# kris927b/TextBlaster

Measured on AMD Instinct MI355X. Metric: documents/sec through full C4+Gopher+langID pipeline at 1/2/4/8 MI355X, higher is better.
Workload: dtype bf16

## Files before the change

### csrc/common/langid.h

```cpp
#pragma once
#include <cmath>

#include "ucd.h"

namespace tb {

constexpr int kLidLangs = 5;
constexpr int kLidRow = 8;
constexpr int kLidBucketsLog2 = 16;
constexpr uint32_t kLidBuckets = 1u << kLidBucketsLog2;
constexpr int kLidMaxCps = 4096;
constexpr int kLidMaxGrams = 4;
constexpr uint32_t kLidBoundary = 0x20;
constexpr int kLidDim = 32;
constexpr int kLidRowDim = 16;
constexpr int kLidHeadCols = 16;
constexpr int kLidQMax = 255;

TB_HD uint32_t lid_hash(uint32_t a, uint32_t b, uint32_t c, uint32_t d, int n) {
  uint32_t h = 2166136261u ^ (uint32_t)n * 0x9E3779B1u;
  h = (h ^ a) * 16777619u;
  if (n >= 2) h = (h ^ b) * 16777619u;
  if (n >= 3) h = (h ^ c) * 16777619u;
  if (n >= 4) h = (h ^ d) * 16777619u;
  h ^= h >> 15;
  h *= 0x2c1b3c6dU;
  h ^= h >> 12;
  return h & (kLidBuckets - 1);
}

template <class F>
TB_HD int lid_grams_n(uint32_t lm3, uint32_t lm2, uint32_t lm1, uint32_t l0, F&& emit) {
  const uint32_t B = kLidBoundary;
  if (l0) {
    emit(lid_hash(l0, 0, 0, 0, 1), 1);
    emit(lid_hash(lm1 ? lm1 : B, l0, 0, 0, 2), 2);
    if (!lm1) return 2;
    emit(lid_hash(lm2 ? lm2 : B, lm1, l0, 0, 3), 3);
    if (!lm2) return 3;
    emit(lid_hash(lm3 ? lm3 : B, lm2, lm1, l0, 4), 4);
    return 4;
  }
  if (!lm1) return 0;
  emit(lid_hash(lm1, B, 0, 0, 2), 2);
  emit(lid_hash(lm2 ? lm2 : B, lm1, B, 0, 3), 3);
  if (!lm2) return 2;
  emit(lid_hash(lm3 ? lm3 : B, lm2, lm1, B, 4), 4);
  return 3;
}

template <class F>
TB_HD int lid_grams_at(uint32_t lm3, uint32_t lm2, uint32_t lm1, uint32_t l0, F&& emit) {
  return lid_grams_n(lm3, lm2, lm1, l0, [&](uint32_t g, int) { emit(g); });
}

TB_HD double lid_exp(double x) {
  if (!(x > -745.0)) return 0.0;
  const double k = floor(fma(x, 1.4426950408889634, 0.5));
  double r = fma(-k, 6.93147180369123816490e-01, x);
  r = fma(-k, 1.90821492927058770002e-10, r);
  double p = 1.0 / 6227020800.0;
  const double inv[13] = {1.0 / 479001600.0, 1.0 / 39916800.0, 1.0 / 3628800.0, 1.0 / 362880.0, 1.0 / 40320.0,
                          1.0 / 5040.0, 1.0 / 720.0, 1.0 / 120.0, 1.0 / 24.0, 1.0 / 6.0, 0.5, 1.0, 1.0};
#pragma unroll
  for (int i = 0; i < 13; ++i) p = fma(p, r, inv[i]);
  return ldexp(p, (int)k);
}

TB_HD void lid_softmax_decide(const double* logit, int64_t* r) {
  int best = 0;
  for (int l = 1; l < kLidLangs; ++l) if (logit[l] > logit[best]) best = l;
  double den = 0;
  for (int l = 0; l < kLidLangs; ++l) den += lid_exp(logit[l] - logit[best]);
  const double conf = 1.0 / den;
  r[0] = best;
  union { double d; int64_t i; } u;
  u.d = conf;
  r[1] = u.i;
}

TB_HD int lid_block_exp(int64_t smax, int64_t cnt) {
  int e = 0;
  while (e < 30 && (smax << (e + 1)) <= (int64_t)kLidQMax * cnt) ++e;
  return e;
}

TB_HD int32_t lid_quant(int64_t s, int e, int64_t cnt) {
  const bool neg = s < 0;
  const int64_t num = (neg ? -s : s) << e;
  int64_t q = num / cnt;
  const int64_t rem = num - q * cnt;
  if (2 * rem > cnt || (2 * rem == cnt && (q & 1))) ++q;
  return (int32_t)(neg ? -q : q);
}

TB_HD void lid_decide_v3(const double* C, int e, int64_t cnt, double w_scale, const float* bias, int64_t* r) {
  if (cnt <= 0) {
    r[0] = -1;
    r[1] = 0;
    return;
  }
  const double sc = ldexp(w_scale, -e);
  double logit[kLidLangs];
  for (int l = 0; l < kLidLangs; ++l) logit[l] = fma(C[l], sc, (double)bias[l]);
  lid_softmax_decide(logit, r);
}

TB_HD uint16_t lid_bf16_bits(float v) {
  union { float f; uint32_t u; } x;
  x.f = v;
  return (uint16_t)(x.u >> 16);
}

TB_HD uint32_t lid_letter(const UcdView& ucd, const uint8_t* b, uint32_t n, int64_t s) {
  if (s < 0) return 0;
  const uint32_t c0 = b[s];
  if (c0 < 0x80u) {
    const uint32_t l = c0 | 0x20u;
    return (l >= 'a' && l <= 'z') ? l : 0u;
  }
  int len;
  const uint32_t c = utf8_decode(b, (uint32_t)s, n, &len);
  if (!(ucd.props(c) & P_ALPHA)) return 0;
  const uint32_t l = ucd.lower(c);
  return l ? l : c;
}

TB_HD int64_t prev_lead(const uint8_t* b, int64_t s) {
  int64_t k = s - 1;
  while (k >= 0 && !utf8_is_lead(b[k])) --k;
  return k;
}

struct LidTables {
  const float* bias = nullptr;
  const int8_t* E = nullptr;
  const int16_t* W = nullptr;
  double w_scale = 0;
};

TB_HD int lid_half(int n) { return n >= 3 ? kLidRowDim : 0; }

TB_HD void lid_add_emb(const int8_t* E, uint32_t g, int n, int32_t* acc) {
  const int8_t* r = E + (size_t)g * kLidRowDim;
  int32_t* a = acc + lid_half(n);
#pragma unroll
  for (int d = 0; d < kLidRowDim; ++d) a[d] += r[d];
}

TB_HD void lid_record_v3(const int64_t* S, int64_t cnt, const LidTables& lt, int64_t* r) {
  if (cnt <= 0) {
    r[0] = -1;
    r[1] = 0;
    return;
  }
  int64_t smax = 0;
  for (int d = 0; d < kLidDim; ++d) smax = (S[d] < 0 ? -S[d] : S[d]) > smax ? (S[d] < 0 ? -S[d] : S[d]) : smax;
  const int e = lid_block_exp(smax, cnt);
  int32_t a[kLidDim];
  for (int d = 0; d < kLidDim; ++d) a[d] = lid_quant(S[d], e, cnt);
  double C[kLidLangs];
  for (int l = 0; l < kLidLangs; ++l) {
    int64_t c = 0;
    for (int d = 0; d < kLidDim; ++d) c += (int64_t)a[d] * lt.W[d * kLidLangs + l];
    C[l] = (double)c;
  }
  lid_decide_v3(C, e, cnt, lt.w_scale, lt.bias, r);
}

}
```

### csrc/hip/langid.hip

```cpp
#include "kernel_common.h"

namespace {

__device__ __forceinline__ int lid_top(uint64_t m) { return 63 - __clzll((long long)m); }

constexpr int kLidTile = 16;
constexpr int kLidWaves = 8;
typedef __bf16 bf16x8 __attribute__((ext_vector_type(8)));
typedef float f32x4 __attribute__((ext_vector_type(4)));

__device__ __forceinline__ void lid_row_swar(const uint8_t* __restrict__ Eb, uint32_t g, uint32_t* p) {
  const uint4 w = *(const uint4*)(Eb + (size_t)g * kLidRowDim);
  const uint32_t v[4] = {w.x, w.y, w.z, w.w};
#pragma unroll
  for (int q = 0; q < 4; ++q) {
    p[2 * q] += v[q] & 0x00FF00FFu;
    p[2 * q + 1] += (v[q] >> 8) & 0x00FF00FFu;
  }
}

constexpr int kLidSyms = 32;
constexpr int kLidPairs = kLidSyms * kLidSyms;
constexpr uint32_t kLidSymMiss = 32;
constexpr int kLidAuxBytes = kLidPairs * 32 + kLidRowDim;

__device__ __forceinline__ uint32_t lid_sym_letter(int i) {
  if (i == 0) return kLidBoundary;
  if (i <= 26) return 'a' + (uint32_t)(i - 1);
  return i == 27 ? 0xE6 : i == 28 ? 0xF8 : i == 29 ? 0xE5 : i == 30 ? 0xE4 : 0xF6;
}

__device__ __forceinline__ uint32_t lid_sym_latin(uint32_t l) {
  return l == 0xE6 ? 27u : l == 0xF8 ? 28u : l == 0xE5 ? 29u : l == 0xE4 ? 30u : l == 0xF6 ? 31u : kLidSymMiss;
}

__global__ __launch_bounds__(256) void k_lid_pairs(const uint8_t* __restrict__ Eb, uint32_t* __restrict__ aux) {
  const int i = (int)(blockIdx.x * blockDim.x + threadIdx.x);
  if (i < kLidPairs) {
    const int x = i / kLidSyms, y = i % kLidSyms;
    uint32_t d[kLidRowDim];
#pragma unroll
    for (int k = 0; k < kLidRowDim; ++k) d[k] = 0;
    auto add = [&](uint32_t g) {
      for (int k = 0; k < kLidRowDim; ++k) d[k] += Eb[(size_t)g * kLidRowDim + k];
    };
    if (y != 0) add(lid_hash(lid_sym_letter(y), 0, 0, 0, 1));
    if (x != 0 || y != 0) add(lid_hash(lid_sym_letter(x), lid_sym_letter(y), 0, 0, 2));
    for (int q = 0; q < 4; ++q) {
      aux[i * 8 + 2 * q] = d[4 * q] | d[4 * q + 2] << 16;
      aux[i * 8 + 2 * q + 1] = d[4 * q + 1] | d[4 * q + 3] << 16;
    }
  }
  if (i < kLidRowDim / 4) aux[kLidPairs * 8 + i] = 0;
}

__device__ __forceinline__ uint32_t lid_letter_dev(uint32_t cur, const uint8_t* b, uint32_t n, uint32_t s,
                                                   const UcdView& ucd) {
  if (cur < 0x80u) return (cur | 0x20u) - 'a' < 26u ? (cur | 0x20u) : 0u;
  if (cur == 0xC3u && s + 1 < n) {
    const uint32_t c = 0xC0u | (b[s + 1] & 0x3Fu);
    return (c == 0xD7u || c == 0xF7u) ? 0u : (c < 0xDFu ? c | 0x20u : c);
  }
  return lid_letter(ucd, b, n, s);
}

__device__ __forceinline__ void lid_add_u8(uint4 w, uint32_t* p) {
  const uint32_t v[4] = {w.x, w.y, w.z, w.w};
#pragma unroll
  for (int q = 0; q < 4; ++q) {
    p[2 * q] += v[q] & 0x00FF00FFu;
    p[2 * q + 1] += (v[q] >> 8) & 0x00FF00FFu;
  }
}

template <int N>
__device__ __forceinline__ void lid_halve(const int32_t* in, int32_t* out, bool upper, int m) {
#pragma unroll
  for (int j = 0; j < N / 2; ++j) {
    const int32_t keep = upper ? in[N / 2 + j] : in[j];
    const int32_t give = upper ? in[j] : in[N / 2 + j];
    out[j] = keep + __shfl_xor(give, m);
  }
}

__device__ __forceinline__ void lid_fold(uint32_t* pa, uint32_t* pb, int lane, int32_t& dsum) {
  const bool up = (lane >> 5) & 1;
  uint32_t kept[8];
#pragma unroll
  for (int j = 0; j < 8; ++j) {
    const uint32_t keep = up ? pb[j] : pa[j];
    const uint32_t give = up ? pa[j] : pb[j];
    kept[j] = keep + (uint32_t)__shfl_xor((int)give, 32);
    pa[j] = pb[j] = 0;
  }
  int32_t u[16], v8[8], v4[4], v2[2], v1;
#pragma unroll
  for (int j = 0; j < 8; ++j) {
    u[2 * j] = (int32_t)(kept[j] & 0xFFFFu);
    u[2 * j + 1] = (int32_t)(kept[j] >> 16);
  }
  lid_halve<16>(u, v8, (lane >> 4) & 1, 16);
  lid_halve<8>(v8, v4, (lane >> 3) & 1, 8);
  lid_halve<4>(v4, v2, (lane >> 2) & 1, 4);
  lid_halve<2>(v2, &v1, (lane >> 1) & 1, 2);
  dsum += v1 + __shfl_xor(v1, 1);
}

__device__ __forceinline__ void lid_doc_vector(const uint8_t* __restrict__ b, uint32_t n, const UcdView& ucd,
                                               const uint8_t* __restrict__ Eb, const uint8_t* __restrict__ zero,
                                               const uint4* pairs, uint32_t* slot, int lane, uint16_t* arow,
                                               int32_t* e_out, int64_t* cnt_out) {
  uint32_t lim = n;
  if (n > (uint32_t)kLidMaxCps) {
    uint32_t seen = 0;
    for (uint32_t base = 0; base < n; base += 64) {
      const uint32_t i = base + (uint32_t)lane;
      const uint64_t m = __ballot(i < n && utf8_is_lead(b[i]));
      const uint32_t c = (uint32_t)__popcll(m);
      if (seen + c > (uint32_t)kLidMaxCps) {
        uint64_t mm = m;
        for (uint32_t k = seen; k < (uint32_t)kLidMaxCps; ++k) mm &= mm - 1;
        lim = base + (uint32_t)__builtin_ctzll(mm);
        break;
      }
      seen += c;
    }
  }
  uint32_t pa[8] = {0u, 0u, 0u, 0u, 0u, 0u, 0u, 0u}, pb[8] = {0u, 0u, 0u, 0u, 0u, 0u, 0u, 0u};
  int32_t dsum = 0;
  uint32_t cnt_lo = 0, cnt_hi = 0, chunks = 0;
  const uint32_t B = kLidBoundary;
  if (lane < 3) slot[lane] = 0;
  uint8_t cur = (uint32_t)lane < lim ? b[lane] : (uint8_t)0;
  for (uint32_t base = 0; base <= lim; base += 64) {
    const uint32_t s = base + (uint32_t)lane;
    const uint8_t nxt = s + 64 < lim ? b[s + 64] : (uint8_t)0;
    const bool lead = s < lim && utf8_is_lead(cur);
    const bool emit = lead || s == lim;
    uint32_t l0 = 0, y = 0;
    if (lead) {
      l0 = lid_letter_dev(cur, b, n, s, ucd);
      y = l0 < 0x80u ? (l0 & 0x1Fu) : lid_sym_latin(l0);
    }
    const uint64_t M = __ballot(lead);
    const uint64_t EM = __ballot(emit);
    const uint32_t r = __builtin_amdgcn_mbcnt_hi((uint32_t)(EM >> 32), __builtin_amdgcn_mbcnt_lo((uint32_t)EM, 0u));
    if (lead) slot[3 + r] = l0 | y << 24;
    __builtin_amdgcn_fence(__ATOMIC_RELEASE, "wavefront");
    __builtin_amdgcn_wave_barrier();
    __builtin_amdgcn_fence(__ATOMIC_ACQUIRE, "wavefront");
    uint32_t e1 = slot[2 + r], e2 = slot[1 + r], e3 = slot[r];
    if (!emit) e1 = e2 = e3 = 0;
    const uint32_t lm1 = e1 & 0xFFFFFFu, lm2 = e2 & 0xFFFFFFu, lm3 = e3 & 0xFFFFFFu;
    const uint32_t x = e1 >> 24;
    const bool miss = ((x | y) & kLidSymMiss) != 0;
    const uint4* pr = pairs + 2 * (miss ? 0u : (x << 5 | y));
    const uint4 t0 = pr[0], t1 = pr[1];
    pa[0] += t0.x; pa[1] += t0.y; pa[2] += t0.z; pa[3] += t0.w;
    pa[4] += t1.x; pa[5] += t1.y; pa[6] += t1.z; pa[7] += t1.w;
    cnt_lo += (l0 != 0u) + ((l0 | lm1) != 0u);
    if (__ballot(miss)) {
      if (miss) {
        if (l0) lid_add_u8(*(const uint4*)(Eb + (size_t)lid_hash(l0, 0, 0, 0, 1) * kLidRowDim), pa);
        if (l0 | lm1)
          lid_add_u8(*(const uint4*)(Eb + (size_t)lid_hash(lm1 ? lm1 : B, l0 ? l0 : B, 0, 0, 2) * kLidRowDim), pa);
      }
    }
    const uint32_t x0 = l0 ? l0 : B;
    const bool v3 = lm1 != 0u, v4 = v3 && lm2 != 0u;
    const uint8_t* g3 = v3 ? Eb + (size_t)lid_hash(lm2 ? lm2 : B, lm1, x0, 0, 3) * kLidRowDim : zero;
    const uint8_t* g4 = v4 ? Eb + (size_t)lid_hash(lm3 ? lm3 : B, lm2, lm1, x0, 4) * kLidRowDim : zero;
    lid_add_u8(*(const uint4*)g3, pb);
    lid_add_u8(*(const uint4*)g4, pb);
    cnt_hi += (uint32_t)v3 + (uint32_t)v4;
    if ((++chunks & 63u) == 0) lid_fold(pa, pb, lane, dsum);
    const uint32_t c = (uint32_t)__popcll(M);
    uint32_t keep = 0;
    if (lane < 3) keep = slot[c + lane];
    __builtin_amdgcn_fence(__ATOMIC_RELEASE, "wavefront");
    __builtin_amdgcn_wave_barrier();
    __builtin_amdgcn_fence(__ATOMIC_ACQUIRE, "wavefront");
    if (lane < 3) slot[lane] = keep;
    cur = nxt;
  }
  lid_fold(pa, pb, lane, dsum);
  for (int o = 1; o < 64; o <<= 1) {
    cnt_lo += (uint32_t)__shfl_xor((int)cnt_lo, o);
    cnt_hi += (uint32_t)__shfl_xor((int)cnt_hi, o);
  }
  const uint32_t cnt = cnt_lo + cnt_hi;
  const bool up = ((lane >> 5) & 1) != 0;
  const int32_t S = dsum - 128 * (int32_t)(up ? cnt_hi : cnt_lo);
  const int dim = ((lane >> 5) & 1) * 16 + (2 * ((lane >> 4) & 1) + ((lane >> 3) & 1)) * 4 + ((lane >> 2) & 1) +
                  2 * ((lane >> 1) & 1);
  int32_t smax = S < 0 ? -S : S;
  for (int o = 1; o < 64; o <<= 1) {
    const int32_t t = __shfl_xor(smax, o);
    smax = t > smax ? t : smax;
  }
  const int e = cnt ? lid_block_exp((int64_t)smax, (int64_t)cnt) : 0;
  if ((lane & 1) == 0) arow[dim] = cnt ? lid_bf16_bits((float)lid_quant((int64_t)S, e, (int64_t)cnt)) : (uint16_t)0;
  if (lane == 0) {
    *e_out = e;
    *cnt_out = (int64_t)cnt;
  }
}

__global__ __launch_bounds__(64 * kLidWaves) __attribute__((amdgpu_waves_per_eu(8, 8))) void k_langid_mfma(
    const uint8_t* __restrict__ bytes, const int64_t* __restrict__ off, const int32_t* __restrict__ perm,
    int32_t ndocs, DevTables tabs, const uint8_t* __restrict__ Eb, const uint8_t* __restrict__ aux,
    const uint16_t* __restrict__ WT, double w_scale, const float* __restrict__ bias, int64_t* rec, int32_t width,
    uint64_t* prof) {
  __shared__ __attribute__((aligned(16))) uint16_t A[kLidTile][kLidDim];
  __shared__ float Cm[kLidTile][kLidHeadCols];
  __shared__ int32_t ex[kLidTile];
  __shared__ int64_t cn[kLidTile];
  __shared__ uint4 pairs[2 * kLidPairs];
  __shared__ uint32_t slots[kLidWaves][68];
  const int w = (int)(threadIdx.x >> 6), lane = (int)(threadIdx.x & 63);
  const UcdView ucd{tabs.s1, tabs.s2, tabs.l1, tabs.l2};
  for (int i = (int)threadIdx.x; i < 2 * kLidPairs; i += 64 * kLidWaves) pairs[i] = ((const uint4*)aux)[i];
  const uint8_t* zero = aux + kLidPairs * 32;
  __syncthreads();
  const int ntiles = (ndocs + kLidTile - 1) / kLidTile;
  for (int tile = (int)blockIdx.x; tile < ntiles; tile += (int)gridDim.x) {
    for (int r = w; r < kLidTile; r += kLidWaves) {
      const int pos = tile * kLidTile + r;
      const int doc = pos < ndocs ? (perm ? perm[pos] : pos) : -1;
      if (doc < 0) {
        if (lane < kLidDim) A[r][lane] = 0;
        if (lane == 0) {
          ex[r] = 0;
          cn[r] = 0;
        }
        continue;
      }
      const uint64_t t0 = prof ? __builtin_amdgcn_s_memtime() : 0;
      lid_doc_vector(bytes + off[doc], (uint32_t)(off[doc + 1] - off[doc]), ucd, Eb, zero, pairs, slots[w], lane,
                     A[r], &ex[r], &cn[r]);
      if (prof && lane == 0) prof[(size_t)doc * kPhaseSlots + PH_LID] += __builtin_amdgcn_s_memtime() - t0;
    }
    __syncthreads();
    if (w == 0) {
      const bf16x8 a = *reinterpret_cast<const bf16x8*>(&A[lane & 15][8 * (lane >> 4)]);
      const bf16x8 bw = *reinterpret_cast<const bf16x8*>(WT + (lane & 15) * kLidDim + 8 * (lane >> 4));
      f32x4 c = {0.f, 0.f, 0.f, 0.f};
      c = __builtin_amdgcn_mfma_f32_16x16x32_bf16(a, bw, c, 0, 0, 0);
#pragma unroll
      for (int r = 0; r < 4; ++r) Cm[(lane >> 4) * 4 + r][lane & 15] = c[r];
      __builtin_amdgcn_fence(__ATOMIC_RELEASE, "workgroup");
      __builtin_amdgcn_wave_barrier();
      __builtin_amdgcn_fence(__ATOMIC_ACQUIRE, "workgroup");
      const int p2 = tile * kLidTile + lane;
      if (lane < kLidTile && p2 < ndocs) {
        const int d2 = perm ? perm[p2] : p2;
        double C[kLidLangs];
#pragma unroll
        for (int l = 0; l < kLidLangs; ++l) C[l] = (double)Cm[lane][l];
        lid_decide_v3(C, ex[lane], cn[lane], w_scale, bias, rec + (int64_t)d2 * width);
      }
    }
    __syncthreads();
  }
}

}

extern "C" {

int tb_langid_aux_bytes() { return kLidAuxBytes; }
int tb_langid_prepare(hipStream_t stream, const uint8_t* E, uint8_t* aux) {
  if (!E || !aux) return (int)hipErrorInvalidValue;
  hipLaunchKernelGGL(k_lid_pairs, dim3((kLidPairs + 255) / 256), dim3(256), 0, stream, E, (uint32_t*)aux);
  return (int)hipGetLastError();
}

int tb_langid_mfma(hipStream_t stream, const TbDocs* d, const TbTables* tb, const uint8_t* E, const uint8_t* aux,
                   const uint16_t* WT, double w_scale, const float* bias, int64_t* rec, int32_t width,
                   uint64_t* prof) {
  const int32_t ndocs = d->n_launch;
  if (ndocs <= 0) return 0;
  if (!E || !aux || !WT || !bias || !rec || width < 2 || !(w_scale > 0)) return (int)hipErrorInvalidValue;
  const int ntiles = (ndocs + kLidTile - 1) / kLidTile;
  const int cus = device_cus();
  const int grid = ntiles < 4 * cus ? ntiles : 4 * cus;
  hipLaunchKernelGGL(k_langid_mfma, dim3(grid), dim3(64 * kLidWaves), 0, stream, d->bytes, d->off, d->perm, ndocs,
                     tb->ucd, E, aux, WT, w_scale, bias, rec, width, prof);
  return (int)hipGetLastError();
}

}
```

Before: 14.13 million.

## Precompute trigram embedding table and rework langid scan with ballot/bpermute and buffer loads

Adds a precomputed 32^3 symbol-trigram table built at prepare time, so most 3-gram hashes become direct table lookups instead of hash plus random embedding gathers. The per-wave LDS slot exchange with barriers is replaced by ds_bpermute/readlane carry of the previous letters. UTF-8 lead detection now uses ballot-mask arithmetic, ASCII and 2-byte letters go through a 256-entry LDS lookup table, and row loads use bounds-checked buffer loads that return zero out of range, which removes the zero-row pointer trick. It also drops the final count shuffle reduction by counting with popcount on masks. The aux buffer grows (32K trigram rows), and the rewritten position logic brings a correctness risk.

```diff
diff --git a/csrc/common/langid.h b/csrc/common/langid.h
--- a/csrc/common/langid.h
+++ b/csrc/common/langid.h
@@ -148,6 +148,40 @@
   for (int d = 0; d < kLidRowDim; ++d) a[d] += r[d];
 }
 
+constexpr int kLidSyms = 32;
+constexpr uint32_t kLidSymMiss = 32;
+
+TB_HD uint32_t lid_sym_letter(int i) {
+  if (i == 0) return kLidBoundary;
+  if (i <= 26) return 'a' + (uint32_t)(i - 1);
+  return i == 27 ? 0xE6 : i == 28 ? 0xF8 : i == 29 ? 0xE5 : i == 30 ? 0xE4 : 0xF6;
+}
+
+TB_HD uint32_t lid_sym_latin(uint32_t l) {
+  return l == 0xE6 ? 27u : l == 0xF8 ? 28u : l == 0xE5 ? 29u : l == 0xE4 ? 30u : l == 0xF6 ? 31u : kLidSymMiss;
+}
+
+TB_HD uint32_t lid_sym(uint32_t l) { return l < 0x80u ? (l & 0x1Fu) : lid_sym_latin(l); }
+
+template <class T>
+TB_HD void lid_pair_entry(const T* E, int x, int y, int32_t* d) {
+  if (y != 0) {
+    const T* r = E + (size_t)lid_hash(lid_sym_letter(y), 0, 0, 0, 1) * kLidRowDim;
+    for (int k = 0; k < kLidRowDim; ++k) d[k] += (int32_t)r[k];
+  }
+  if (x != 0 || y != 0) {
+    const T* r = E + (size_t)lid_hash(lid_sym_letter(x), lid_sym_letter(y), 0, 0, 2) * kLidRowDim;
+    for (int k = 0; k < kLidRowDim; ++k) d[k] += (int32_t)r[k];
+  }
+}
+
+template <class T>
+TB_HD void lid_tri_entry(const T* E, int s2, int s1, int s0, int32_t* d) {
+  if (s1 == 0) return;
+  const T* r = E + (size_t)lid_hash(lid_sym_letter(s2), lid_sym_letter(s1), lid_sym_letter(s0), 0, 3) * kLidRowDim;
+  for (int k = 0; k < kLidRowDim; ++k) d[k] += (int32_t)r[k];
+}
+
 TB_HD void lid_record_v3(const int64_t* S, int64_t cnt, const LidTables& lt, int64_t* r) {
   if (cnt <= 0) {
     r[0] = -1;
diff --git a/csrc/hip/langid.hip b/csrc/hip/langid.hip
--- a/csrc/hip/langid.hip
+++ b/csrc/hip/langid.hip
@@ -1,6 +1,12 @@
 #include "kernel_common.h"
 
 namespace {
+
+__device__ __forceinline__ uint64_t lid_eq(uint32_t a, uint32_t b) { return __builtin_amdgcn_uicmp(a, b, 32); }
+__device__ __forceinline__ uint64_t lid_ne(uint32_t a, uint32_t b) { return __builtin_amdgcn_uicmp(a, b, 33); }
+__device__ __forceinline__ uint64_t lid_lt(uint32_t a, uint32_t b) { return __builtin_amdgcn_uicmp(a, b, 36); }
+__device__ __forceinline__ uint64_t lid_ge(uint32_t a, uint32_t b) { return __builtin_amdgcn_uicmp(a, b, 35); }
+__device__ __forceinline__ bool lid_on(uint64_t m) { return __builtin_amdgcn_inverse_ballot_w64(m); }
 
 __device__ __forceinline__ int lid_top(uint64_t m) { return 63 - __clzll((long long)m); }
 
@@ -9,49 +15,45 @@
 typedef __bf16 bf16x8 __attribute__((ext_vector_type(8)));
 typedef float f32x4 __attribute__((ext_vector_type(4)));
 
-__device__ __forceinline__ void lid_row_swar(const uint8_t* __restrict__ Eb, uint32_t g, uint32_t* p) {
-  const uint4 w = *(const uint4*)(Eb + (size_t)g * kLidRowDim);
-  const uint32_t v[4] = {w.x, w.y, w.z, w.w};
-#pragma unroll
-  for (int q = 0; q < 4; ++q) {
-    p[2 * q] += v[q] & 0x00FF00FFu;
-    p[2 * q + 1] += (v[q] >> 8) & 0x00FF00FFu;
-  }
-}
-
-constexpr int kLidSyms = 32;
+#ifndef TB_LID_TRI_ROW
+#define TB_LID_TRI_ROW 16
+#endif
+constexpr int kLidTriRow = TB_LID_TRI_ROW;
+static_assert(kLidTriRow == 32 || kLidTriRow == 16, "3-gram row: 32 (pre-split) or 16 (bytes)");
 constexpr int kLidPairs = kLidSyms * kLidSyms;
-constexpr uint32_t kLidSymMiss = 32;
-constexpr int kLidAuxBytes = kLidPairs * 32 + kLidRowDim;
-
-__device__ __forceinline__ uint32_t lid_sym_letter(int i) {
-  if (i == 0) return kLidBoundary;
-  if (i <= 26) return 'a' + (uint32_t)(i - 1);
-  return i == 27 ? 0xE6 : i == 28 ? 0xF8 : i == 29 ? 0xE5 : i == 30 ? 0xE4 : 0xF6;
-}
-
-__device__ __forceinline__ uint32_t lid_sym_latin(uint32_t l) {
-  return l == 0xE6 ? 27u : l == 0xF8 ? 28u : l == 0xE5 ? 29u : l == 0xE4 ? 30u : l == 0xF6 ? 31u : kLidSymMiss;
-}
-
-__global__ __launch_bounds__(256) void k_lid_pairs(const uint8_t* __restrict__ Eb, uint32_t* __restrict__ aux) {
+constexpr int kLidTris = kLidSyms * kLidSyms * kLidSyms;
+constexpr int kLidZeroOff = kLidPairs * 32;
+constexpr int kLidTriOff = kLidZeroOff + 32;
+constexpr int kLidAuxBytes = kLidTriOff + kLidTris * kLidTriRow;
+
+__global__ __launch_bounds__(256) void k_lid_tables(const uint8_t* __restrict__ Eb, uint32_t* __restrict__ aux) {
   const int i = (int)(blockIdx.x * blockDim.x + threadIdx.x);
+  if (i >= kLidPairs + kLidTris) return;
+  int32_t d[kLidRowDim];
+#pragma unroll
+  for (int k = 0; k < kLidRowDim; ++k) d[k] = 0;
+  uint32_t* out;
+  bool split = true;
   if (i < kLidPairs) {
-    const int x = i / kLidSyms, y = i % kLidSyms;
-    uint32_t d[kLidRowDim];
-#pragma unroll
-    for (int k = 0; k < kLidRowDim; ++k) d[k] = 0;
-    auto add = [&](uint32_t g) {
-      for (int k = 0; k < kLidRowDim; ++k) d[k] += Eb[(size_t)g * kLidRowDim + k];
-    };
-    if (y != 0) add(lid_hash(lid_sym_letter(y), 0, 0, 0, 1));
-    if (x != 0 || y != 0) add(lid_hash(lid_sym_letter(x), lid_sym_letter(y), 0, 0, 2));
+    lid_pair_entry(Eb, i / kLidSyms, i % kLidSyms, d);
+    out = aux + i * 8;
+  } else {
+    const int t = i - kLidPairs;
+    lid_tri_entry(Eb, t / kLidPairs, (t / kLidSyms) % kLidSyms, t % kLidSyms, d);
+    out = aux + kLidTriOff / 4 + t * (kLidTriRow / 4);
+    split = kLidTriRow == 32;
+  }
+  if (split) {
     for (int q = 0; q < 4; ++q) {
-      aux[i * 8 + 2 * q] = d[4 * q] | d[4 * q + 2] << 16;
-      aux[i * 8 + 2 * q + 1] = d[4 * q + 1] | d[4 * q + 3] << 16;
-    }
-  }
-  if (i < kLidRowDim / 4) aux[kLidPairs * 8 + i] = 0;
+      out[2 * q] = (uint32_t)d[4 * q] | (uint32_t)d[4 * q + 2] << 16;
+      out[2 * q + 1] = (uint32_t)d[4 * q + 1] | (uint32_t)d[4 * q + 3] << 16;
+    }
+  } else {
+    for (int q = 0; q < 4; ++q)
+      out[q] = (uint32_t)d[4 * q] | (uint32_t)d[4 * q + 1] << 8 | (uint32_t)d[4 * q + 2] << 16 |
+               (uint32_t)d[4 * q + 3] << 24;
+  }
+  if (i < (kLidTriOff - kLidZeroOff) / 4) aux[kLidZeroOff / 4 + i] = 0;
 }
 
 __device__ __forceinline__ uint32_t lid_letter_dev(uint32_t cur, const uint8_t* b, uint32_t n, uint32_t s,
@@ -64,13 +66,77 @@
   return lid_letter(ucd, b, n, s);
 }
 
+__device__ __forceinline__ uint32_t lid_table_entry(uint32_t i, uint32_t* buf, const UcdView& ucd) {
+  const uint32_t c0 = i < 0x80u ? i : (0xC2u | ((i >> 6) & 1u));
+  *buf = c0 | (0x80u | (i & 0x3Fu)) << 8;
+  const uint32_t l = lid_letter_dev(c0, (const uint8_t*)buf, i < 0x80u ? 1u : 2u, 0u, ucd);
+  return l ? (l | lid_sym(l) << 24) : 0u;
+}
+
+constexpr uint32_t kLidNoRow = 0x7FFFFFF0u;
+__device__ __forceinline__ __amdgpu_buffer_rsrc_t lid_rsrc(const uint8_t* p, uint32_t bytes) {
+  return __builtin_amdgcn_make_buffer_rsrc((void*)p, 0, (int)bytes, 0x00027000);
+}
+__device__ __forceinline__ uint4 lid_row(__amdgpu_buffer_rsrc_t r, uint32_t off) {
+  typedef uint32_t u32x4 __attribute__((ext_vector_type(4)));
+  const u32x4 v = __builtin_amdgcn_raw_buffer_load_b128(r, (int)off, 0, 0);
+  return uint4{v.x, v.y, v.z, v.w};
+}
+
+__device__ __forceinline__ uint32_t lid_byte(__amdgpu_buffer_rsrc_t r, uint32_t off) {
+  return __builtin_amdgcn_raw_buffer_load_b8(r, (int)off, 0, 0);
+}
+
+__device__ __forceinline__ uint64_t lid_low(int32_t r) {
+  return r >= 64 ? ~(uint64_t)0 : r <= 0 ? (uint64_t)0 : (((uint64_t)1 << r) - 1);
+}
+
+__device__ __forceinline__ uint64_t lid_positions(uint32_t cur, uint64_t K1, int32_t left, uint64_t& pend) {
+  const uint64_t in = lid_low(left);
+  const uint64_t L2 = lid_eq(cur & 0xE0u, 0xC0u) & lid_low(left - 1);
+  const uint64_t L3 = lid_eq(cur & 0xF0u, 0xE0u) & lid_low(left - 2);
+  const uint64_t L4 = ~(K1 | L2 | L3) & lid_low(left - 3);
+  uint64_t P = in & lid_ne(cur & 0xC0u, 0x80u);
+  uint64_t a = P & (L2 | L3 | L4), b = P & (L3 | L4), c = P & L4;
+  if ((in & ~(pend | a << 1 | b << 2 | c << 3)) != P) {
+    uint64_t cov = pend;
+    P = 0;
+    for (int i = 0; i < 64; ++i) {
+      const uint64_t bit = (uint64_t)1 << i;
+      if (in & ~cov & bit) {
+        P |= bit;
+        cov |= ((L2 | L3 | L4) & bit) << 1 | ((L3 | L4) & bit) << 2 | (L4 & bit) << 3;
+      }
+    }
+    a = P & (L2 | L3 | L4), b = P & (L3 | L4), c = P & L4;
+  }
+  pend = a >> 63 | b >> 62 | c >> 61;
+  return P;
+}
+
 __device__ __forceinline__ void lid_add_u8(uint4 w, uint32_t* p) {
   const uint32_t v[4] = {w.x, w.y, w.z, w.w};
+  uint32_t even, odd;
+  asm("s_mov_b32 %0, 0x0c020c00" : "=s"(even));
+  asm("s_mov_b32 %0, 0x0c030c01" : "=s"(odd));
 #pragma unroll
   for (int q = 0; q < 4; ++q) {
-    p[2 * q] += v[q] & 0x00FF00FFu;
-    p[2 * q + 1] += (v[q] >> 8) & 0x00FF00FFu;
-  }
+    p[2 * q] += __builtin_amdgcn_perm(0u, v[q], even);
+    p[2 * q + 1] += __builtin_amdgcn_perm(0u, v[q], odd);
+  }
+}
+
+__device__ __forceinline__ void lid_add_split(uint4 t0, uint4 t1, uint32_t* p) {
+  p[0] += t0.x; p[1] += t0.y; p[2] += t0.z; p[3] += t0.w;
+  p[4] += t1.x; p[5] += t1.y; p[6] += t1.z; p[7] += t1.w;
+}
+
+__device__ __forceinline__ void lid_add_rows(uint4 r3a, uint4 r3b, uint4 r4, uint32_t* pb) {
+  if (kLidTriRow == 32)
+    lid_add_split(r3a, r3b, pb);
+  else
+    lid_add_u8(r3a, pb);
+  lid_add_u8(r4, pb);
 }
 
 template <int N>
@@ -107,15 +173,19 @@
 }
 
 __device__ __forceinline__ void lid_doc_vector(const uint8_t* __restrict__ b, uint32_t n, const UcdView& ucd,
-                                               const uint8_t* __restrict__ Eb, const uint8_t* __restrict__ zero,
-                                               const uint4* pairs, uint32_t* slot, int lane, uint16_t* arow,
-                                               int32_t* e_out, int64_t* cnt_out) {
+                                               const uint8_t* __restrict__ Eb,
+                                               __amdgpu_buffer_rsrc_t EbR, __amdgpu_buffer_rsrc_t triR,
+                                               const uint4* pairs,
+                                               const uint32_t* ltab, int lane, uint16_t* arow, int32_t* e_out,
+                                               int64_t* cnt_out) {
   uint32_t lim = n;
   if (n > (uint32_t)kLidMaxCps) {
     uint32_t seen = 0;
+    uint64_t pend = 0;
     for (uint32_t base = 0; base < n; base += 64) {
       const uint32_t i = base + (uint32_t)lane;
-      const uint64_t m = __ballot(i < n && utf8_is_lead(b[i]));
+      const uint32_t ci = i < n ? b[i] : 0u;
+      const uint64_t m = lid_positions(ci, lid_lt(ci, 0x80u), (int32_t)(n - base), pend);
       const uint32_t c = (uint32_t)__popcll(m);
       if (seen + c > (uint32_t)kLidMaxCps) {
         uint64_t mm = m;
@@ -125,69 +195,94 @@
       }
       seen += c;
     }
+    lim = (uint32_t)__builtin_amdgcn_readfirstlane((int)lim);
   }
   uint32_t pa[8] = {0u, 0u, 0u, 0u, 0u, 0u, 0u, 0u}, pb[8] = {0u, 0u, 0u, 0u, 0u, 0u, 0u, 0u};
   int32_t dsum = 0;
   uint32_t cnt_lo = 0, cnt_hi = 0, chunks = 0;
+  uint32_t c1 = 0, c2 = 0, c3 = 0;
+  uint64_t pend = 0;
   const uint32_t B = kLidBoundary;
-  if (lane < 3) slot[lane] = 0;
-  uint8_t cur = (uint32_t)lane < lim ? b[lane] : (uint8_t)0;
+  const uint64_t below = ((uint64_t)1 << lane) - 1;
+  const __amdgpu_buffer_rsrc_t docR = lid_rsrc(b, n);
+  uint32_t cur = lid_byte(docR, (uint32_t)lane);
+  uint32_t n0 = lid_byte(docR, 64u);
   for (uint32_t base = 0; base <= lim; base += 64) {
-    const uint32_t s = base + (uint32_t)lane;
-    const uint8_t nxt = s + 64 < lim ? b[s + 64] : (uint8_t)0;
-    const bool lead = s < lim && utf8_is_lead(cur);
-    const bool emit = lead || s == lim;
-    uint32_t l0 = 0, y = 0;
-    if (lead) {
-      l0 = lid_letter_dev(cur, b, n, s, ucd);
-      y = l0 < 0x80u ? (l0 & 0x1Fu) : lid_sym_latin(l0);
-    }
-    const uint64_t M = __ballot(lead);
-    const uint64_t EM = __ballot(emit);
-    const uint32_t r = __builtin_amdgcn_mbcnt_hi((uint32_t)(EM >> 32), __builtin_amdgcn_mbcnt_lo((uint32_t)EM, 0u));
-    if (lead) slot[3 + r] = l0 | y << 24;
-    __builtin_amdgcn_fence(__ATOMIC_RELEASE, "wavefront");
-    __builtin_amdgcn_wave_barrier();
-    __builtin_amdgcn_fence(__ATOMIC_ACQUIRE, "wavefront");
-    uint32_t e1 = slot[2 + r], e2 = slot[1 + r], e3 = slot[r];
-    if (!emit) e1 = e2 = e3 = 0;
-    const uint32_t lm1 = e1 & 0xFFFFFFu, lm2 = e2 & 0xFFFFFFu, lm3 = e3 & 0xFFFFFFu;
-    const uint32_t x = e1 >> 24;
-    const bool miss = ((x | y) & kLidSymMiss) != 0;
-    const uint4* pr = pairs + 2 * (miss ? 0u : (x << 5 | y));
-    const uint4 t0 = pr[0], t1 = pr[1];
-    pa[0] += t0.x; pa[1] += t0.y; pa[2] += t0.z; pa[3] += t0.w;
-    pa[4] += t1.x; pa[5] += t1.y; pa[6] += t1.z; pa[7] += t1.w;
-    cnt_lo += (l0 != 0u) + ((l0 | lm1) != 0u);
-    if (__ballot(miss)) {
-      if (miss) {
+    const uint32_t cur1 = lid_byte(docR, base + 64u + (uint32_t)lane);
+    const uint32_t n01 = lid_byte(docR, base + 128u);
+    const int32_t rem = (int32_t)(lim - base);
+    const int32_t left = (int32_t)(n - base);
+    const uint64_t AS = lid_lt(cur, 0x80u);
+    uint64_t P;
+    {
+      const uint64_t A = lid_ge(cur, 0xC0u), E3 = lid_ge(cur, 0xE0u), F4 = lid_ge(cur, 0xF0u);
+      if (left >= 67 && (pend | A << 1 | E3 << 2 | F4 << 3) == ~(AS | A)) {
+        P = AS | A;
+        pend = A >> 63 | E3 >> 62 | F4 >> 61;
+      } else {
+        P = lid_positions(cur, AS, left, pend);
+      }
+    }
+    const uint64_t M = P & lid_low(rem);
+    const uint64_t EM = M | (lid_low(rem + 1) & ~lid_low(rem));
+    uint32_t nb = lane_next(cur);
+    if (lane == 63) nb = n0;
+    const uint64_t TW = lid_eq(cur & 0xFEu, 0xC2u) & lid_low(left - 1);
+    const uint32_t i2 = ((cur << 6 | (nb & 0x3Fu)) & 0x7Fu) | 0x80u;
+    uint32_t ent = ltab[lid_on(M & AS) ? cur : (lid_on(M & TW) ? i2 : 0u)];
+    const uint64_t G = M & ~AS & ~TW;
+    if (G) {
+      if (lid_on(G)) {
+        const uint32_t l = lid_letter(ucd, b, n, base + (uint32_t)lane);
+        ent = l ? (l | lid_sym(l) << 24) : 0u;
+      }
+    }
+    const uint64_t pm = M & below;
+    const bool hasp = pm != 0;
+    const int pl = (63 - __clzll((long long)pm)) << 2;
+    uint32_t e1 = (uint32_t)__builtin_amdgcn_ds_bpermute(pl, (int)ent);
+    e1 = hasp ? e1 : c1;
+    uint32_t e2 = (uint32_t)__builtin_amdgcn_ds_bpermute(pl, (int)e1);
+    e2 = hasp ? e2 : c2;
+    uint32_t e3 = (uint32_t)__builtin_amdgcn_ds_bpermute(pl, (int)e2);
+    e3 = hasp ? e3 : c3;
+    if (M) {
+      const int t = lid_top(M);
+      c3 = (uint32_t)__builtin_amdgcn_readlane((int)e2, t);
+      c2 = (uint32_t)__builtin_amdgcn_readlane((int)e1, t);
+      c1 = (uint32_t)__builtin_amdgcn_readlane((int)ent, t);
+    }
+    e1 = lid_on(EM) ? e1 : 0u;
+    const uint32_t l0 = ent & 0xFFFFFFu, lm1 = e1 & 0xFFFFFFu, lm2 = e2 & 0xFFFFFFu, lm3 = e3 & 0xFFFFFFu;
+    const uint32_t y = ent >> 24, x = e1 >> 24, s2 = e2 >> 24;
+    const uint64_t L0 = lid_ne(l0, 0u), L1 = lid_ne(lm1, 0u), V4 = L1 & lid_ne(lm2, 0u);
+    const uint64_t MS = lid_ne((x | y) & kLidSymMiss, 0u), MS3 = lid_ne((x | y | s2) & kLidSymMiss, 0u);
+    const uint32_t pi = x << 5 | y;
+    const uint4* pr = pairs + 2 * (lid_on(MS) ? 0u : pi);
+    const uint32_t g3 = (s2 << 10 | pi) * (uint32_t)kLidTriRow;
+    const uint32_t x0 = lid_on(L0) ? l0 : B;
+    const uint32_t g4 = lid_hash(lm3 ? lm3 : B, lm2, lm1, x0, 4) * (uint32_t)kLidRowDim;
+    uint4 q3b = {0u, 0u, 0u, 0u};
+    const uint4 q3a = lid_row(triR, lid_on(L1 & ~MS3) ? g3 : kLidNoRow);
+    if (kLidTriRow == 32) q3b = lid_row(triR, lid_on(L1 & ~MS3) ? g3 + 16u : kLidNoRow);
+    const uint4 q4 = lid_row(EbR, lid_on(V4) ? g4 : kLidNoRow);
+    lid_add_split(pr[0], pr[1], pa);
+    lid_add_rows(q3a, q3b, q4, pb);
+    cnt_lo += (uint32_t)__popcll(L0) + (uint32_t)__popcll(L0 | L1);
+    cnt_hi += (uint32_t)__popcll(L1) + (uint32_t)__popcll(V4);
+    if (MS3) {
+      if (lid_on(MS)) {
         if (l0) lid_add_u8(*(const uint4*)(Eb + (size_t)lid_hash(l0, 0, 0, 0, 1) * kLidRowDim), pa);
         if (l0 | lm1)
-          lid_add_u8(*(const uint4*)(Eb + (size_t)lid_hash(lm1 ? lm1 : B, l0 ? l0 : B, 0, 0, 2) * kLidRowDim), pa);
-      }
-    }
-    const uint32_t x0 = l0 ? l0 : B;
-    const bool v3 = lm1 != 0u, v4 = v3 && lm2 != 0u;
-    const uint8_t* g3 = v3 ? Eb + (size_t)lid_hash(lm2 ? lm2 : B, lm1, x0, 0, 3) * kLidRowDim : zero;
-    const uint8_t* g4 = v4 ? Eb + (size_t)lid_hash(lm3 ? lm3 : B, lm2, lm1, x0, 4) * kLidRowDim : zero;
-    lid_add_u8(*(const uint4*)g3, pb);
-    lid_add_u8(*(const uint4*)g4, pb);
-    cnt_hi += (uint32_t)v3 + (uint32_t)v4;
+          lid_add_u8(*(const uint4*)(Eb + (size_t)lid_hash(lm1 ? lm1 : B, x0, 0, 0, 2) * kLidRowDim), pa);
+      }
+      if (lid_on(MS3 & L1)) lid_add_u8(*(const uint4*)(Eb + (size_t)lid_hash(lm2 ? lm2 : B, lm1, x0, 0, 3) * kLidRowDim), pb);
+    }
     if ((++chunks & 63u) == 0) lid_fold(pa, pb, lane, dsum);
-    const uint32_t c = (uint32_t)__popcll(M);
-    uint32_t keep = 0;
-    if (lane < 3) keep = slot[c + lane];
-    __builtin_amdgcn_fence(__ATOMIC_RELEASE, "wavefront");
-    __builtin_amdgcn_wave_barrier();
-    __builtin_amdgcn_fence(__ATOMIC_ACQUIRE, "wavefront");
-    if (lane < 3) slot[lane] = keep;
-    cur = nxt;
+    cur = cur1;
+    n0 = n01;
   }
   lid_fold(pa, pb, lane, dsum);
-  for (int o = 1; o < 64; o <<= 1) {
-    cnt_lo += (uint32_t)__shfl_xor((int)cnt_lo, o);
-    cnt_hi += (uint32_t)__shfl_xor((int)cnt_hi, o);
-  }
   const uint32_t cnt = cnt_lo + cnt_hi;
   const bool up = ((lane >> 5) & 1) != 0;
   const int32_t S = dsum - 128 * (int32_t)(up ? cnt_hi : cnt_lo);
@@ -204,6 +299,14 @@
     *e_out = e;
     *cnt_out = (int64_t)cnt;
   }
+}
+
+__device__ __noinline__ void lid_decide_row(const float* c, int e, int64_t cnt, double w_scale, const float* bias,
+                                            int64_t* r) {
+  double C[kLidLangs];
+#pragma unroll
+  for (int l = 0; l < kLidLangs; ++l) C[l] = (double)c[l];
+  lid_decide_v3(C, e, cnt, w_scale, bias, r);
 }
 
 __global__ __launch_bounds__(64 * kLidWaves) __attribute__((amdgpu_waves_per_eu(8, 8))) void k_langid_mfma(
@@ -216,11 +319,16 @@
   __shared__ int32_t ex[kLidTile];
   __shared__ int64_t cn[kLidTile];
   __shared__ uint4 pairs[2 * kLidPairs];
-  __shared__ uint32_t slots[kLidWaves][68];
-  const int w = (int)(threadIdx.x >> 6), lane = (int)(threadIdx.x & 63);
+  __shared__ uint32_t ltab[256];
+  const int w = __builtin_amdgcn_readfirstlane((int)(threadIdx.x >> 6)), lane = (int)(threadIdx.x & 63);
   const UcdView ucd{tabs.s1, tabs.s2, tabs.l1, tabs.l2};
   for (int i = (int)threadIdx.x; i < 2 * kLidPairs; i += 64 * kLidWaves) pairs[i] = ((const uint4*)aux)[i];
-  const uint8_t* zero = aux + kLidPairs * 32;
+  if (threadIdx.x < 256) {
+    const uint32_t ent = lid_table_entry(threadIdx.x, &ltab[threadIdx.x], ucd);
+    ltab[threadIdx.x] = ent;
+  }
+  const __amdgpu_buffer_rsrc_t EbR = lid_rsrc(Eb, kLidBuckets * kLidRowDim);
+  const __amdgpu_buffer_rsrc_t triR = lid_rsrc(aux + kLidTriOff, (uint32_t)kLidTris * kLidTriRow);
   __syncthreads();
   const int ntiles = (ndocs + kLidTile - 1) / kLidTile;
   for (int tile = (int)blockIdx.x; tile < ntiles; tile += (int)gridDim.x) {
@@ -236,7 +344,7 @@
         continue;
       }
       const uint64_t t0 = prof ? __builtin_amdgcn_s_memtime() : 0;
-      lid_doc_vector(bytes + off[doc], (uint32_t)(off[doc + 1] - off[doc]), ucd, Eb, zero, pairs, slots[w], lane,
+      lid_doc_vector(bytes + off[doc], (uint32_t)(off[doc + 1] - off[doc]), ucd, Eb, EbR, triR, pairs, ltab, lane,
                      A[r], &ex[r], &cn[r]);
       if (prof && lane == 0) prof[(size_t)doc * kPhaseSlots + PH_LID] += __builtin_amdgcn_s_memtime() - t0;
     }
@@ -254,10 +362,7 @@
       const int p2 = tile * kLidTile + lane;
       if (lane < kLidTile && p2 < ndocs) {
         const int d2 = perm ? perm[p2] : p2;
-        double C[kLidLangs];
-#pragma unroll
-        for (int l = 0; l < kLidLangs; ++l) C[l] = (double)Cm[lane][l];
-        lid_decide_v3(C, ex[lane], cn[lane], w_scale, bias, rec + (int64_t)d2 * width);
+        lid_decide_row(Cm[lane], ex[lane], cn[lane], w_scale, bias, rec + (int64_t)d2 * width);
       }
     }
     __syncthreads();
@@ -271,7 +376,8 @@
 int tb_langid_aux_bytes() { return kLidAuxBytes; }
 int tb_langid_prepare(hipStream_t stream, const uint8_t* E, uint8_t* aux) {
   if (!E || !aux) return (int)hipErrorInvalidValue;
-  hipLaunchKernelGGL(k_lid_pairs, dim3((kLidPairs + 255) / 256), dim3(256), 0, stream, E, (uint32_t*)aux);
+  hipLaunchKernelGGL(k_lid_tables, dim3((kLidPairs + kLidTris + 255) / 256), dim3(256), 0, stream, E,
+                     (uint32_t*)aux);
   return (int)hipGetLastError();
 }
 
```

New measurement: 14.16 million, median of 3. About the same (+0.2%).
